# VachaLab/gorder

Hardware: AMD Instinct MI355X
Metric: trajectory frames/sec (higher is better)
Workload: dtype f32

## Files before the change

gorder_amd/csrc/gorder_hip.hip:

```cpp
#include <hip/hip_runtime.h>

#include <dlfcn.h>

#include <cmath>
#include <cstdio>
#include <cstdlib>
#include <cstring>
#include <mutex>
#include <new>
#include <string>
#include <deque>
#include <type_traits>
#include <vector>

#include "../../include/gorder_hip.h"
#include "gm_math.h"
#include "plan.h"
#include "collect_store.h"
#include "device_mem.h"
#include "replay_rows.h"
#include "leaflet_rows.h"
#include "timewise_blocks.h"
#include "ordermap_final.h"
#include "order_route.h"
// ... 135 lines not shown
    DBuf<Item> d_items_by_slot;
    DBuf<uint32_t> d_ua_item_run, d_item_run;
    DBuf<uint4> d_lgrid;
    DBuf<LocalRowPre> d_lrowpre;
    DBuf<LocalEdge> d_ledge;
    DBuf<float4> d_lfinfo;
    static constexpr uint32_t kDecidePause = 16;
    DBuf<uint32_t> d_lsummary;
    HBuf<uint32_t> h_lsummary;
    Event lsummary_written;
    bool lsummary_pending = false;
    uint32_t decide_pause = 0;
    uint64_t decide_submits = 0, decide_paused_submits = 0;
    DBuf<uint32_t> d_lneed;
    DBuf<uint2> d_ltodo;
    size_t map_lds_bytes = 0;
    bool map_staged = false;
    uint64_t map_pending = 0;
    uint32_t map_max_mol = 1;
    DBuf<u64> d_tw_sums, d_tw_cnts;
    uint64_t tw_cap = 0;
    DBuf<u64> d_twx_blocks, d_twx_rows, d_twx_totals, d_twx_edge;
    DBuf<uint32_t> d_twx_groups;
    DBuf<float> d_twx_out;
    DBuf<uint32_t> d_omx_groups;
    DBuf<float> d_omx_out;
    ExtraArgs extra{};
    DBuf<uint32_t> d_geom_group;
    DBuf<float> d_shapes;
    DBuf<float> d_inv_box;
// ... 311 lines not shown
int fold_maps(gorder_hip_handle *h) {
    if (!h->extra.maps || !h->map_pending) return GORDER_OK;
    const size_t n = (size_t)h->plan.n_acc * h->map_nx * h->map_ny;
    const uint32_t blocks = (uint32_t)std::min<size_t>((n + 255) / 256, 256 * 16);
    hipLaunchKernelGGL(k_fold_maps, dim3(blocks), dim3(256), 0, h->stream, h->d_map_packed, h->d_map_sums, h->d_map_cnts,
                       n, h->tables.leaflets.method != GORDER_LEAFLETS_NONE ? 1 : 0);
    HIP_TRY(h, hipGetLastError());
    h->map_pending = 0;
    return GORDER_OK;
}

int launch_cell_list(gorder_hip_handle *h, const LocalArgs &lo, uint32_t ns, uint32_t n_list, void *counts, size_t count_bytes) {
    const bool three = h->sw.local_three_kernels;
    TIMING_MARK(h, n_list <= kLocalBuildMax && !three ? "k_local_build" : "k_local_bin + k_local_scan + k_local_scatter");
    if (n_list <= kLocalBuildMax && !three) {
        if (n_list <= 2u * 8192u) hipLaunchKernelGGL(k_local_build<2>, dim3(ns), dim3(1024), kLocalBuildLds, h->stream, lo);
        else if (n_list <= 5u * 8192u) hipLaunchKernelGGL(k_local_build<5>, dim3(ns), dim3(1024), kLocalBuildLds, h->stream, lo);
        else hipLaunchKernelGGL(k_local_build<kLocalBuildTrips>, dim3(ns), dim3(1024), kLocalBuildLds, h->stream, lo);
        return GORDER_OK;
    }
    HIP_TRY(h, hipMemsetAsync(counts, 0, count_bytes, h->stream));
    const dim3 ga((n_list + 255) / 256, ns);
    hipLaunchKernelGGL(k_local_bin, ga, dim3(256), 0, h->stream, lo);
    hipLaunchKernelGGL(k_local_scan, dim3(ns), dim3(1024), 0, h->stream, lo);
    hipLaunchKernelGGL(k_local_scatter, ga, dim3(256), 0, h->stream, lo);
    return GORDER_OK;
}

int run_dynamic_normals(gorder_hip_handle *h, const FrameArgs &a) {
    int st;
    const uint32_t n_mol = h->plan.n_mol_total;
    if ((st = ensure(h, h->d_dyn_normals, (size_t)a.n_frames * n_mol)) != GORDER_OK) return st;
    const gorder_dynamic_normal_t &dn = h->tables.dynamic_normal;
// ... 961 lines not shown
    const size_t nm = t->leaflets.n_membrane, ncell = (size_t)kLocalMaxCells1D * kLocalMaxCells1D;
    const size_t sl = h->local_slab = local_slab_frames(nm, h->sw.local_slab);
    ST_TRY(local_build_attributes(h));
    h->local_halo = t->handle_pbc && !h->sw.local_atoms_only;
    h->local_rec_stride = (h->local_halo ? 2u : 1u) * nm;
    ST_TRY(allocate(h, h->d_lcell_of, sl * nm));
    ST_TRY(allocate(h, h->d_ltrig, sl * h->local_rec_stride * (sizeof(LocalRec) / sizeof(float))));
    ST_TRY(allocate(h, h->d_lcell_count, sl * (ncell + 1)));
    ST_TRY(allocate(h, h->d_lcell_fill, sl * ncell));
    ST_TRY(allocate(h, h->d_lgrid, sl));
    if (!h->local_halo) return GORDER_OK;
    const size_t row_cells = sl * (size_t)kLocalMaxCells1D * (kLocalMaxCells1D + 1u);
    ST_TRY(allocate(h, h->d_lrowpre, row_cells));
    ST_TRY(allocate(h, h->d_ledge, row_cells));
    ST_TRY(allocate(h, h->d_lfinfo, sl));
    ST_TRY(allocate(h, h->d_lneed, sl + 1));
    ST_TRY(allocate(h, h->d_lsummary, 2, 0));
    ST_TRY(allocate(h, h->h_lsummary, 2));
    h->h_lsummary[0] = h->h_lsummary[1] = 0u;
    HIP_TRY(h, h->lsummary_written.create());
    HIP_TRY(h, hipFuncSetAttribute(reinterpret_cast<const void *>(k_local_decide), hipFuncAttributeMaxDynamicSharedMemorySize, (int)kDecideLds));
    HIP_TRY(h, hipFuncSetAttribute(reinterpret_cast<const void *>(k_local_sums), hipFuncAttributeMaxDynamicSharedMemorySize, (int)kSumsLds));
    return allocate(h, h->d_ltodo, 1 + sl * (size_t)(p.n_mol_total ? p.n_mol_total : 1));
}

int gorder_hip_create(const gorder_tables_t *t, gorder_hip_handle **out) {
    if (!t || !out) return GORDER_ERR_INVALID_ARGUMENT;
    *out = nullptr;
    int n_dev = 0;
    if (hipGetDeviceCount(&n_dev) != hipSuccess || n_dev <= 0) return GORDER_ERR_NO_DEVICE;
    if (t->device < 0 || t->device >= n_dev) return GORDER_ERR_INVALID_ARGUMENT;
// ... 344 lines not shown
    return d;
}

static int launch_local_slabs(gorder_hip_handle *h, LocalArgs lo, uint32_t n_assign, uint32_t row0, bool report) {
    const size_t ncell = (size_t)kLocalMaxCells1D * kLocalMaxCells1D;
    for (size_t done = 0; done < n_assign; done += h->local_slab) {
        const uint32_t ns = (uint32_t)std::min<size_t>(n_assign - done, h->local_slab);
        lo.aframes = h->d_aframes + done;
        lo.n_slab = ns;
        lo.row0 = row0 + (uint32_t)done;
        lo.write_dist_frame = (done + ns == n_assign) ? (int)ns - 1 : -1;
        lo.summary_host = report && done + ns == n_assign ? h->h_lsummary : nullptr;
        if (lo.n_membrane > kLocalBuildMax || h->sw.local_three_kernels)
            HIP_TRY(h, hipMemsetAsync(h->d_lcell_fill, 0, ns * ncell * sizeof(uint32_t), h->stream));
        if (lo.sums) {
            HIP_TRY(h, hipMemsetAsync(h->d_lneed, 0, (ns + 1) * sizeof(uint32_t), h->stream));
            TIMING_MARK(h, "k_local_sums");
            hipLaunchKernelGGL(k_local_sums, dim3(ns), dim3(1024), kSumsLds, h->stream, lo);
            TIMING_MARK(h, "k_local_decide");
            hipLaunchKernelGGL(k_local_decide, dim3(ns), dim3(1024), kDecideLds, h->stream, lo);
        }
        ST_TRY(launch_cell_list(h, lo, ns, lo.n_membrane, h->d_lcell_count, ns * (ncell + 1) * sizeof(uint32_t)));
        if (lo.halo) {
            TIMING_MARK(h, "k_local_rowprefix");
            hipLaunchKernelGGL(k_local_rowprefix, dim3(kLocalMaxCells1D / 4u, ns), dim3(256), 0, h->stream, lo);
            lo.rows_groups = (lo.n_mol_total + 15u) / 16u;
            if (lo.need && !lo.sums) {
                TIMING_MARK(h, "k_local_decide");
                hipLaunchKernelGGL(k_local_decide, dim3(ns), dim3(1024), kDecideLds, h->stream, lo);
            }
            TIMING_MARK(h, "k_local_flags_rows");
            if (lo.need) hipLaunchKernelGGL(k_local_flags_rows_open, dim3(lo.rows_groups * 8u * kRowsSlots), dim3(256), 0, h->stream, lo);
            else hipLaunchKernelGGL(k_local_flags_rows, dim3(lo.rows_groups * ((ns + 7u) / 8u * 8u)), dim3(256), 0, h->stream, lo);
            TIMING_MARK(h, "k_local_flags_todo");
            hipLaunchKernelGGL(k_local_flags_todo, dim3(512), dim3(256), 0, h->stream, lo);
        } else {
            TIMING_MARK(h, "k_local_flags");
            hipLaunchKernelGGL(k_local_flags, dim3((lo.n_mol_total + 3) / 4, ns), dim3(256), 0, h->stream, lo);
        }
    }
// ... 12 lines not shown
    lo.radius_thr = local_radius_threshold(lf.radius);
    lo.cell_of = h->d_lcell_of; lo.trig = h->d_ltrig; lo.cell_count = h->d_lcell_count;
    lo.cell_fill = h->d_lcell_fill; lo.err = la.err;
    lo.grid = h->d_lgrid;
    lo.halo = h->local_halo ? 1 : 0;
    lo.prune = h->sw.local_no_prune ? 0 : (h->sw.local_decide_nothing ? 2 : 1);
    lo.rec_stride = (uint32_t)h->local_rec_stride;
    lo.rowpre = h->d_lrowpre;
    lo.edge = h->d_ledge;
    lo.finfo = h->d_lfinfo;
    lo.todo = h->d_ltodo;
    const LocalDecisions d = local_decisions(h, lo);
    lo.need = d.decide ? h->d_lneed : nullptr;
    lo.sums = d.sums ? 1 : 0;
    lo.summary = d.report ? h->d_lsummary : nullptr;
    ST_TRY(launch_local_slabs(h, lo, la.n_assign, la.row0, d.report));
    if (d.report) {
        HIP_TRY(h, hipEventRecord(h->lsummary_written, h->stream));
        h->lsummary_pending = true;
    }
    return GORDER_OK;
}

static int run_leaflets(gorder_hip_handle *h, const float *d_xyz, const float *d_box,
                        const std::vector<uint32_t> &aframes, uint32_t row0, const uint8_t *skip = nullptr) {
    if (aframes.empty()) return GORDER_OK;
    ST_TRY(upload_if_changed(h, h->d_aframes, h->up_aframes, h->up_aframes_valid, aframes));
    const gorder_leaflets_t &lf = h->tables.leaflets;
    LeafletArgs la{};
    la.xyz = d_xyz; la.box9 = d_box; la.n_atoms = h->plan.n_atoms;
// ... 1252 lines not shown
int gorder_hip_collected_normals(gorder_hip_handle *h, float *normals, uint64_t *frames, uint64_t capacity_rows, uint64_t *n_rows) {
    if (!h || !n_rows) return GORDER_ERR_INVALID_ARGUMENT;
    *n_rows = 0;
    if (!(h->collect & GORDER_COLLECT_NORMALS)) return fail(h, GORDER_ERR_INVALID_ARGUMENT, "gorder_hip_collected_normals: normals are not being collected");
    const gorder::CollectStore &store = h->collect_normals;
    *n_rows = store.n_rows();
    if ((normals || frames) && capacity_rows < store.n_rows()) return fail(h, GORDER_ERR_INVALID_ARGUMENT, "gorder_hip_collected_normals: capacity_rows is too small");
    ST_TRY(gorder_hip_synchronize(h));
    const size_t row_floats = (size_t)h->plan.n_mol_total * 3u;
    if (normals)
        store.for_each_row([&](uint64_t r, const void *row) { memcpy(normals + r * row_floats, row, row_floats * sizeof(float)); });
    if (frames && store.n_rows()) memcpy(frames, store.frames().data(), store.n_rows() * sizeof(uint64_t));
    return GORDER_OK;
}

int gorder_hip_leaflet_distances(gorder_hip_handle *h, float *dist) {
    if (!h || !dist || !h->d_adist) return GORDER_ERR_INVALID_ARGUMENT;
    ST_TRY(gorder_hip_synchronize(h));
    HIP_TRY(h, hipMemcpy(dist, h->d_adist, sizeof(float) * h->plan.n_mol_total, hipMemcpyDeviceToHost));
    return GORDER_OK;
}

int gorder_hip_spherical_stats(gorder_hip_handle *h, float out[12]) {
    if (!h || !out || h->tables.leaflets.method != GORDER_LEAFLETS_SPHERICAL || !h->d_sph_stats) return GORDER_ERR_INVALID_ARGUMENT;
    if (!h->have_assignment) return fail(h, GORDER_ERR_INVALID_ARGUMENT, "gorder_hip_spherical_stats: no assignment frame yet");
    ST_TRY(gorder_hip_synchronize(h));
    HIP_TRY(h, hipMemcpy(out, h->d_sph_stats, 12 * sizeof(float), hipMemcpyDeviceToHost));
    return GORDER_OK;
}

int gorder_hip_clustering_stats(gorder_hip_handle *h, float out[12]) {
    if (!h || !out || h->tables.leaflets.method != GORDER_LEAFLETS_CLUSTERING || !h->d_cl_stats) return GORDER_ERR_INVALID_ARGUMENT;
    if (!h->have_assignment) return fail(h, GORDER_ERR_INVALID_ARGUMENT, "gorder_hip_clustering_stats: no assignment frame yet");
// ... 74 lines not shown
    h->mol_batch_log.clear();
    h->collect_locked = false;
    h->have_assignment = false;
    h->cl_have_carry = false;
    h->replay_have_carry = false;
    h->assignment_frame = 0;
    h->manual_frames = 0;
    h->err_index = 0;
    h->err_msg.clear();
    if (h->d_own) {
        spec_poll(h, true);
        h->spec_enabled = true;
        h->spec_batches = h->spec_fixed = h->spec_exact_frames = 0;
        HIP_TRY(h, hipMemsetAsync(h->d_spec_counters, 0, 4 * sizeof(uint32_t), h->stream));
    }
    if (h->d_lsummary) {
        if (h->lsummary_pending) { (void)hipEventSynchronize(h->lsummary_written); h->lsummary_pending = false; }
        h->decide_pause = 0;
        h->decide_submits = h->decide_paused_submits = 0;
        h->h_lsummary[0] = h->h_lsummary[1] = 0u;
        HIP_TRY(h, hipMemsetAsync(h->d_lsummary, 0, 2 * sizeof(uint32_t), h->stream));
    }
    return GORDER_OK;
}

int gorder_hip_comm_unique_id(uint8_t id[128]) {
    if (!id) return GORDER_ERR_INVALID_ARGUMENT;
    RcclApi *api = rccl_api(nullptr);
    if (!api) return GORDER_ERR_DEVICE;
    UniqueId u;
// ... 152 lines not shown
```

gorder_amd/csrc/kernels_leaflets.h:

```cpp
#pragma once

namespace {

struct LeafletArgs {
    const float *xyz;
    const float *box9;
    uint32_t n_atoms;
    const uint32_t *aframes;
    uint32_t row0;
    uint8_t *aflags;
    float *adist;
    uint32_t n_mol_total;
    const uint32_t *heads;
    const uint32_t *membrane;
    uint32_t n_membrane;
    const uint32_t *methyl_begin;
    const uint32_t *methyl_atoms;
    uint32_t dim;
    int flip, pbc;
    uint32_t *err;
    const uint8_t *skip;
    uint32_t n_assign;
};

// ... 539 lines not shown
    float *trig;
    uint32_t *cell_count;
    uint32_t *cell_fill;
    int halo;
    int prune;
    uint32_t rows_groups;
    uint32_t rec_stride;
    LocalEdge *edge;
    LocalRowPre *rowpre;
    float4 *finfo;
    uint2 *todo;
    int sums;
    uint32_t *summary;
    uint32_t *summary_host;
    uint32_t *need;
    uint32_t *err;
};

constexpr uint32_t kLocalFine = 4;
constexpr uint32_t kLocalFineRows = 7;
__device__ __forceinline__ void local_axis(float L, float radius, uint32_t &nc, uint32_t &k, uint32_t k_max = kLocalFine,
                                           uint32_t nc_max = kLocalMaxCells1D) {
    nc = 1; k = 0;
    for (uint32_t kk = k_max; kk >= 1u; kk--) {
        const float fine = floorf(L / (radius / (float)kk) * 0.9999f);
        if (fine >= (float)(2u * kk + 1u) && fine <= (float)nc_max) { nc = (uint32_t)fine; k = kk; return; }
    }
}
__device__ __forceinline__ void local_grid(const LocalArgs &a, const float *box, uint32_t &nca, uint32_t &ncb,
                                           int &da, int &db, uint32_t &ka, uint32_t &kb) {
    da = (int)((a.dim + 1u) % 3u);
// ... 252 lines not shown
        if (qb == qa) break;
    }
}
__device__ __forceinline__ void local_finfo_merge(const LocalArgs &a, uint32_t s, float zlo, float zhi, uint32_t nf) {
    wave_minmax_or_bfly(zlo, zhi, nf);
    if ((threadIdx.x & 63u) == 0u) {
        uint32_t *fi = reinterpret_cast<uint32_t *>(a.finfo + s);
        if (zlo <= zhi) {
            atomicMin(fi, local_float_key(zlo));
            atomicMax(fi + 1, local_float_key(zhi));
        }
        if (nf) atomicOr(fi + 2, 1u);
    }
}
constexpr uint32_t kRowPrefixPiece = 256;
__global__ __launch_bounds__(256) void k_local_rowprefix(LocalArgs a) {
    __shared__ alignas(16) float l_c[4][kRowPrefixPiece + 4], l_s[4][kRowPrefixPiece + 4], l_q[4][kRowPrefixPiece + 4];
    __shared__ alignas(16) double l_z[4][kRowPrefixPiece + 2];
    const uint32_t s = blockIdx.y, wave = threadIdx.x >> 6, ra = blockIdx.x * 4u + wave;
    const uint4 g = a.grid[s];
    const uint32_t nca = g.x, ncs = local_row_stride(a, g.y, g.w);
    if (a.sums) {
        if (a.need[a.n_slab] == 0u || a.need[s] == 0u) return;
    } else if (blockIdx.x == 0 && s == 0 && threadIdx.x == 0) a.todo[0] = make_uint2(0u, 0u);
    if (!a.sums && blockIdx.x == 0 && threadIdx.x == 0 && a.need) {
        a.need[s] = 0u;
        if (s == 0) a.need[a.n_slab] = 0u;
    }
    if (ra >= nca) return;
    const bool merge = reinterpret_cast<const uint4 *>(a.finfo)[s].w != 2u;
    const uint32_t *cstart = a.cell_count + (size_t)s * (kLocalMaxCells1D * kLocalMaxCells1D + 1u);
    const LocalRec *rec = reinterpret_cast<const LocalRec *>(a.trig) + (size_t)s * a.rec_stride;
    float box[3];
    frame_box(a, a.aframes ? a.aframes[s] : a.frame0 + s, box);
    LocalRowPre *out = a.rowpre + (size_t)s * (kLocalMaxCells1D * (kLocalMaxCells1D + 1u)) + (size_t)ra * (ncs + 1u);
    LocalEdge *out_edge = a.edge + (size_t)s * (kLocalMaxCells1D * (kLocalMaxCells1D + 1u)) + (size_t)ra * (ncs + 1u);
    float zlo = 3.0e38f, zhi = -3.0e38f;
    uint32_t nf = 0;
    local_row_prefix<kRowPrefixPiece>(cstart, rec, out, out_edge, ra, ncs, 1.0f / box[a.dim], 0.5f * box[a.dim], l_c[wave], l_s[wave], l_z[wave],
                                      l_q[wave], zlo, zhi, nf);
    if (merge) local_finfo_merge(a, s, zlo, zhi, nf);
}

constexpr uint32_t kLocalBuildMax = 65536;
constexpr uint32_t kLocalBuildLds = 2u * kLocalMaxCells1D * kLocalMaxCells1D * (uint32_t)sizeof(uint32_t);
constexpr uint32_t kLocalBuildTrips = kLocalBuildMax / (8u * 1024u);
template <uint32_t TRIPS>
__global__ __launch_bounds__(1024) void k_local_build(LocalArgs a) {
    extern __shared__ uint32_t l_build[];
    __shared__ uint32_t l_wave[16];
    __shared__ uint32_t l_over;
    uint32_t *l_start = l_build, *l_fill = l_build + kLocalMaxCells1D * kLocalMaxCells1D;
    const uint32_t s = blockIdx.x, tid = threadIdx.x;
    if (a.sums && (a.need[a.n_slab] == 0u || a.need[s] == 0u)) return;
    const uint32_t f = a.aframes ? a.aframes[s] : a.frame0 + s;
    float box[3];
    frame_box(a, f, box);
    uint32_t nca, ncb, ka, kb;
    int da, db;
    local_grid(a, box, nca, ncb, da, db, ka, kb);
    const uint32_t ncs = local_row_stride(a, ncb, kb), ncell = nca * ncs;
    const uint32_t n_halo = a.halo ? 2u * kb : 0u;
    const int dn = (int)a.dim;
    for (uint32_t k = tid; k < ncell; k += 1024u) { l_start[k] = 0; l_fill[k] = 0; }
    if (tid == 0) l_over = 0;
    __syncthreads();
    const float *x = a.xyz + (size_t)f * a.n_atoms * 3u;
    int bad = 0;
    bool in_halo = false;
    const float inv_a = a.pbc ? (float)nca / box[da] : 0.0f, inv_b = a.pbc ? (float)ncb / box[db] : 0.0f;
    auto cell_ab = [&](float xa, float xb) -> uint32_t {
        in_halo = false;
        if (!a.pbc) return 0u;
        const float La = box[da], Lb = box[db];
        float wa = xa > La ? xa - La : xa, wb = xb > Lb ? xb - Lb : xb;
        wa = wa < 0.0f ? wa + La : wa;
        wb = wb < 0.0f ? wb + Lb : wb;
        if (__builtin_expect(!(wa >= 0.0f && wa <= La && wb >= 0.0f && wb <= Lb), 0)) {
            wa = gm_wrap(xa, La, bad);
            wb = gm_wrap(xb, Lb, bad);
        }
        const uint32_t ca = (uint32_t)fminf(fmaxf(floorf(wa * inv_a), 0.0f), (float)(nca - 1u));
        const uint32_t cb = (uint32_t)fminf(fmaxf(floorf(wb * inv_b), 0.0f), (float)(ncb - 1u));
        in_halo = cb < n_halo;
        return ca * ncs + cb;
    };
    constexpr uint32_t U = 8;
    uint32_t place[TRIPS][2], place2[TRIPS][2];
    uint32_t cells[TRIPS][4];
    bool over = false;
#pragma unroll
    for (uint32_t trip = 0; trip < TRIPS; trip++) {
        const uint32_t i0 = tid + trip * U * 1024u;
        place[trip][0] = place[trip][1] = place2[trip][0] = place2[trip][1] = 0u;
        cells[trip][0] = cells[trip][1] = cells[trip][2] = cells[trip][3] = 0u;
        if (trip * U * 1024u >= a.n_membrane) continue;
        uint32_t at[U];
        float pa[U], pb[U];
#pragma unroll
        for (uint32_t u = 0; u < U; u++) { const uint32_t i = min(i0 + u * 1024u, a.n_membrane - 1u); at[u] = a.membrane ? a.membrane[i] : i; }
#pragma unroll
        for (uint32_t u = 0; u < U; u++) { pa[u] = x[3u * (size_t)at[u] + da]; pb[u] = x[3u * (size_t)at[u] + db]; }
#pragma unroll
        for (uint32_t u = 0; u < U; u++)
            if (i0 + u * 1024u < a.n_membrane) {
                const uint32_t c = cell_ab(pa[u], pb[u]);
                cells[trip][u >> 1] |= (c | (in_halo ? 0x4000u : 0u)) << (16u * (u & 1u));
                const uint32_t r = atomicAdd(&l_start[c], 1u);
                over |= r > 255u;
                place[trip][u >> 2] |= (r & 255u) << (8u * (u & 3u));
                if (in_halo) {
                    const uint32_t r2 = atomicAdd(&l_start[c + ncb], 1u);
                    over |= r2 > 255u;
                    place2[trip][u >> 2] |= (r2 & 255u) << (8u * (u & 3u));
                }
            }
    }
    if (over) l_over = 1u;
    __syncthreads();
    const bool use_fill = l_over != 0u;
    {
        constexpr uint32_t PER = kLocalMaxCells1D * kLocalMaxCells1D / 1024u;
        const uint32_t c0 = tid * PER;
        uint32_t cnt[PER], sum = 0;
#pragma unroll
        for (uint32_t k = 0; k < PER; k++) {
            cnt[k] = c0 + k < ncell ? l_start[c0 + k] : 0u;
            sum += cnt[k];
        }
        const uint32_t incl = wave_scan_shfl(sum, tid & 63u);
        if ((tid & 63u) == 63u) l_wave[tid >> 6] = incl;
        __syncthreads();
        uint32_t run = incl - sum;
        for (uint32_t w = 0; w < (tid >> 6); w++) run += l_wave[w];
        uint32_t *cstart = a.cell_count + (size_t)s * (kLocalMaxCells1D * kLocalMaxCells1D + 1u);
#pragma unroll
        for (uint32_t k = 0; k < PER; k++) {
            if (c0 + k <= ncell) {
                cstart[c0 + k] = run;
                if (c0 + k < ncell) l_start[c0 + k] = run;
            }
            run += cnt[k];
        }
        if (tid == 1023u && c0 + PER == ncell) cstart[ncell] = run;
    }
    if (tid == 0 && a.grid) { a.grid[s] = make_uint4(nca, ncb, ka, kb); local_finfo_init(a, s); }
    __syncthreads();
    LocalRec *rec = reinterpret_cast<LocalRec *>(a.trig) + (size_t)s * a.rec_stride;
    float zlo = 3.0e38f, zhi = -3.0e38f;
    uint32_t nf = 0;
#pragma unroll
    for (uint32_t trip = 0; trip < TRIPS; trip++) {
        const uint32_t i0 = tid + trip * U * 1024u;
        if (trip * U * 1024u >= a.n_membrane) continue;
        uint32_t at[U];
        float pa[U], pb[U], pn[U];
#pragma unroll
        for (uint32_t u = 0; u < U; u++) { const uint32_t i = min(i0 + u * 1024u, a.n_membrane - 1u); at[u] = a.membrane ? a.membrane[i] : i; }
#pragma unroll
        for (uint32_t u = 0; u < U; u++) {
            pa[u] = x[3u * (size_t)at[u] + da]; pb[u] = x[3u * (size_t)at[u] + db]; pn[u] = x[3u * (size_t)at[u] + dn];
        }
#pragma unroll
        for (uint32_t u = 0; u < U; u++) {
            if (i0 + u * 1024u >= a.n_membrane) continue;
            const uint32_t cw = (cells[trip][u >> 1] >> (16u * (u & 1u))) & 0xffffu;
            const uint32_t c = cw & 0x3fffu;
            in_halo = (cw & 0x4000u) != 0u;
            const uint32_t q = l_start[c] + (use_fill ? atomicAdd(&l_fill[c], 1u) : (place[trip][u >> 2] >> (8u * (u & 3u))) & 255u);
            rec[q] = LocalRec{pa[u], pb[u], pn[u]};
            zlo = fminf(zlo, pn[u]);
            zhi = fmaxf(zhi, pn[u]);
            nf |= ((pa[u] - pa[u]) + (pb[u] - pb[u])) + (pn[u] - pn[u]) == 0.0f ? 0u : 1u;
            if (in_halo) {
                const uint32_t q2 = l_start[c + ncb] + (use_fill ? atomicAdd(&l_fill[c + ncb], 1u) : (place2[trip][u >> 2] >> (8u * (u & 3u))) & 255u);
                rec[q2] = LocalRec{pa[u], pb[u], pn[u]};
            }
        }
    }
    if (bad) raise_box_range(a.err, f);
    if (a.finfo) {
        __shared__ float l_zlo[16], l_zhi[16];
        __shared__ uint32_t l_nf[16];
        block_finfo_record(zlo, zhi, nf, ~0u, l_zlo, l_zhi, l_nf, reinterpret_cast<uint4 *>(a.finfo) + s);
    }
}

__host__ __device__ inline float local_radius_threshold(float r) {
    if (!(r > 0.0f)) return 0.0f;
    float thr = r * r;
    for (int i = 0; i < 8 && sqrtf(thr) < r; i++) thr = nextafterf(thr, INFINITY);
    for (int i = 0; i < 8; i++) {
        const float p = nextafterf(thr, 0.0f);
        if (!(p < thr) || !(sqrtf(p) >= r)) break;
        thr = p;
    }
    return thr;
}

// ... 451 lines not shown
        a.todo[1u + at] = make_uint2(s, m);
    }
}
constexpr uint32_t kRowsSlots = 1;
__global__ __launch_bounds__(256) void k_local_flags_rows(LocalArgs a) {
    __shared__ LocalRingLists l_ring[16];
    const uint32_t n_groups = a.rows_groups, linear = blockIdx.x;
    const uint32_t xcd = linear & 7u, k = linear >> 3;
    const uint32_t s = (k / n_groups) * 8u + xcd, bx = k - (k / n_groups) * n_groups;
    if (s < a.n_slab) local_rows_group(a, s, bx, l_ring);
}
__global__ __launch_bounds__(256) void k_local_flags_rows_open(LocalArgs a) {
    __shared__ LocalRingLists l_ring[16];
    const uint32_t n_groups = a.rows_groups, linear = blockIdx.x;
    const uint32_t xcd = linear & 7u, k = linear >> 3;
    if (a.need[a.n_slab] == 0u) return;
    const uint32_t slot = k / n_groups, bx = k - slot * n_groups, lane = threadIdx.x & 63u;
    uint32_t seen = 0;
    for (uint32_t base = xcd; base < a.n_slab; base += 8u * 64u) {
        const uint32_t sl = base + 8u * lane;
        uint64_t open = __ballot(sl < a.n_slab && a.need[sl] != 0u);
        while (open != 0ull) {
            const uint32_t bit = (uint32_t)__builtin_ctzll(open);
            open &= open - 1ull;
            if (seen++ % kRowsSlots == slot) local_rows_group(a, (uint32_t)__builtin_amdgcn_readfirstlane((int)(base + 8u * bit)), bx, l_ring);
        }
    }
}

constexpr uint32_t kSumsCells = 9000;
constexpr uint32_t kSumsLds = kSumsCells * 2u * (uint32_t)sizeof(unsigned long long);
struct LocalWrapped { float a, b; int bad; };
// ... 193 lines not shown
    const float mid = T - 0.5f * A, rad = 0.5005f * __builtin_amdgcn_sqrtf(fr * B);
    const float slack = 0.1f + fn * (1.05e-3f + 1e-6f * fn * Ln);
    const float r_c = __builtin_amdgcn_sqrtf(c_c * c_c + c_s * c_s);
    const float est_c = (local_atan2_fast(-c_s, -c_c) + 3.1415927f) * (Ln * 0.15915494f);
    const float shift_c = gm_min_image(hn_pos - est_c, Ln, bad);
    const float e_c = fr + 1.0f + 0.004f * fn;
    const float xr = e_c * __builtin_amdgcn_rcpf(r_c);
    const float emargin = 1e-4f * Ln + (xr + 0.5708f * xr * xr * xr) * (0.15916f * Ln);
    const bool same_image = e_c < r_c && ulo_g + shift_c > -halfn + emargin && uhi_g + shift_c < halfn - emargin;
    const bool head_near = __builtin_fabsf(mid) + rad < (halfn - 1e-3f * Ln) * fi;
    centre_above = mid > 0.0f;
    return !redo && spans_ok && c_n > r_n && same_image && head_near && a.prune != 2 &&
           __builtin_fabsf(mid) > rad + slack;
}
template <typename EdgePtr>
__device__ __forceinline__ void local_decide_frame(const LocalArgs &a, const DecideFrame &F, uint32_t s, uint32_t f, EdgePtr edge) {
    int bad = 0;
    uint32_t n_open = 0;
    for (uint32_t m0 = threadIdx.x & ~63u; m0 < a.n_mol_total; m0 += 1024u) {
        const uint32_t m_raw = m0 + (threadIdx.x & 63u);
        const bool head_ok = m_raw < a.n_mol_total;
        const uint32_t m = head_ok ? m_raw : a.n_mol_total - 1u;
        bool centre_above;
        const bool decided = local_decide_head(a, F, f, m, edge, centre_above, bad);
        if (decided && head_ok)
            a.aflags[(size_t)(a.row0 + s) * a.n_mol_total + m] = (uint8_t)((centre_above ? 1 : 0) ^ (a.flip ? 1 : 0));
        n_open += (uint32_t)__popcll(__ballot(!decided && head_ok));
    }
    if (n_open != 0u && (threadIdx.x & 63u) == 0u) { atomicAdd(&a.need[s], n_open); a.need[a.n_slab] = 1u; }
    if (bad) raise_box_range(a.err, f);
}
__global__ __launch_bounds__(1024) void k_local_decide(LocalArgs a) {
    extern __shared__ LocalEdge l_edge[];
    const uint32_t s = blockIdx.x;
    const uint32_t f = a.aframes ? a.aframes[s] : a.frame0 + s;
    float box[3];
    frame_box(a, f, box);
    const uint4 g = a.grid[s];
    const uint4 fk = reinterpret_cast<const uint4 *>(a.finfo)[s];
    DecideFrame F;
    F.nca = g.x; F.ncb = g.y; F.ka = g.z; F.kb = g.w; F.ncs = g.y + 2u * g.w; F.n_rows = 2u * g.z + 1u;
    F.da = (int)((a.dim + 1u) % 3u); F.db = (int)((a.dim + 2u) % 3u); F.dn = (int)a.dim;
    F.La = box[F.da]; F.Lb = box[F.db]; F.Ln = box[F.dn];
    F.z_min = local_key_float(fk.x); F.z_max = local_key_float(fk.y);
    const bool fail = !(F.ka >= 1u && F.kb >= 1u && F.n_rows <= 16u && fk.z == 0u && fk.x <= fk.y);
    if (a.sums && s == 0u && threadIdx.x == 0u) a.todo[0] = make_uint2(0u, 0u);
    if (fail || !(F.z_max - F.z_min < 0.75f * F.Ln) || (int)s == a.write_dist_frame || (a.sums && a.need[s] != 0u)) {
        if (threadIdx.x == 0u) { atomicAdd(&a.need[s], 1u); a.need[a.n_slab] = 1u; }
        return;
    }
    const LocalEdge *edge = a.edge + (size_t)s * (kLocalMaxCells1D * (kLocalMaxCells1D + 1u));
    const uint32_t n_entries = F.nca * (F.ncs + 1u);
    if (n_entries <= kDecideEntries) {
        const uint4 *src = reinterpret_cast<const uint4 *>(edge);
        uint4 *dst = reinterpret_cast<uint4 *>(l_edge);
        for (uint32_t i = threadIdx.x; i < n_entries; i += 1024u) dst[i] = src[i];
        __syncthreads();
        local_decide_frame<const LocalEdge *>(a, F, s, f, l_edge);
    } else {
        local_decide_frame<const LocalEdge *>(a, F, s, f, edge);
    }
}

__global__ __launch_bounds__(256) void k_local_flags_todo(LocalArgs a) {
    if (a.need && a.summary && blockIdx.x == 0u && threadIdx.x < 64u) {
        uint32_t c = 0;
        for (uint32_t s = threadIdx.x; s < a.n_slab; s += 64u) c += a.need[s] != 0u ? 1u : 0u;
        c = wave_sum_rows(c);
        if (threadIdx.x == 0u) {
            const uint32_t open = atomicAdd(&a.summary[0], c) + c, seen = atomicAdd(&a.summary[1], a.n_slab) + a.n_slab;
            if (a.summary_host) {
                a.summary_host[0] = open;
                a.summary_host[1] = seen;
                a.summary[0] = a.summary[1] = 0u;
            }
        }
    }
    const uint32_t n = a.todo[0].x;
    for (uint32_t i = blockIdx.x * 4u + (threadIdx.x >> 6); i < n; i += gridDim.x * 4u) {
        const uint2 e = a.todo[1u + i];
        local_flags_head(a, (uint32_t)__builtin_amdgcn_readfirstlane((int)e.x), (uint32_t)__builtin_amdgcn_readfirstlane((int)e.y));
    }
}

// ... 251 lines not shown
```

Before: 20.96 million.

## Compact open frames into a worklist and defer last-frame distance computation

The decide kernel now appends frames that still need work to a compact list, and the build, rowprefix and rows kernels loop over that list with a capped grid instead of launching one block per slab frame and early-exiting. The last frame of each slab is no longer forced through the full path just to produce leaflet distances. Its coordinates and box are snapshotted on device, and the distances are recomputed lazily only when the host asks for them. This cuts idle blocks and redundant full-path work per batch, at the cost of extra state, a coordinate copy per batch, and added complexity in the query path.

```diff
diff --git a/gorder_amd/csrc/gorder_hip.hip b/gorder_amd/csrc/gorder_hip.hip
--- a/gorder_amd/csrc/gorder_hip.hip
+++ b/gorder_amd/csrc/gorder_hip.hip
@@ -173,6 +173,11 @@
     uint64_t decide_submits = 0, decide_paused_submits = 0;
     DBuf<uint32_t> d_lneed;
     DBuf<uint2> d_ltodo;
+    DBuf<float> d_lkeep_xyz, d_lkeep_box;
+    DBuf<uint32_t> d_lkeep_state, d_lkeep_err;
+    DBuf<uint8_t> d_lkeep_flags;
+    LocalArgs lkeep_args{};
+    bool ldist_maybe_owed = false;
     size_t map_lds_bytes = 0;
     bool map_staged = false;
     uint64_t map_pending = 0;
@@ -514,9 +519,10 @@
     const bool three = h->sw.local_three_kernels;
     TIMING_MARK(h, n_list <= kLocalBuildMax && !three ? "k_local_build" : "k_local_bin + k_local_scan + k_local_scatter");
     if (n_list <= kLocalBuildMax && !three) {
-        if (n_list <= 2u * 8192u) hipLaunchKernelGGL(k_local_build<2>, dim3(ns), dim3(1024), kLocalBuildLds, h->stream, lo);
-        else if (n_list <= 5u * 8192u) hipLaunchKernelGGL(k_local_build<5>, dim3(ns), dim3(1024), kLocalBuildLds, h->stream, lo);
-        else hipLaunchKernelGGL(k_local_build<kLocalBuildTrips>, dim3(ns), dim3(1024), kLocalBuildLds, h->stream, lo);
+        const dim3 grid(lo.open ? std::min(ns, kOpenBuildGroups) : ns);
+        if (n_list <= 2u * 8192u) hipLaunchKernelGGL(k_local_build<2>, grid, dim3(1024), kLocalBuildLds, h->stream, lo);
+        else if (n_list <= 5u * 8192u) hipLaunchKernelGGL(k_local_build<5>, grid, dim3(1024), kLocalBuildLds, h->stream, lo);
+        else hipLaunchKernelGGL(k_local_build<kLocalBuildTrips>, grid, dim3(1024), kLocalBuildLds, h->stream, lo);
         return GORDER_OK;
     }
     HIP_TRY(h, hipMemsetAsync(counts, 0, count_bytes, h->stream));
@@ -1508,7 +1514,12 @@
     ST_TRY(allocate(h, h->d_lrowpre, row_cells));
     ST_TRY(allocate(h, h->d_ledge, row_cells));
     ST_TRY(allocate(h, h->d_lfinfo, sl));
-    ST_TRY(allocate(h, h->d_lneed, sl + 1));
+    ST_TRY(allocate(h, h->d_lneed, 2 * sl + 2));
+    ST_TRY(allocate(h, h->d_lkeep_xyz, (size_t)p.n_atoms * 3u));
+    ST_TRY(allocate(h, h->d_lkeep_box, 9, 0));
+    ST_TRY(allocate(h, h->d_lkeep_state, 1, 0));
+    ST_TRY(allocate(h, h->d_lkeep_err, kErrWords, 0xff));
+    ST_TRY(allocate(h, h->d_lkeep_flags, p.n_mol_total ? p.n_mol_total : 1));
     ST_TRY(allocate(h, h->d_lsummary, 2, 0));
     ST_TRY(allocate(h, h->h_lsummary, 2));
     h->h_lsummary[0] = h->h_lsummary[1] = 0u;
@@ -1883,7 +1894,8 @@
         if (lo.n_membrane > kLocalBuildMax || h->sw.local_three_kernels)
             HIP_TRY(h, hipMemsetAsync(h->d_lcell_fill, 0, ns * ncell * sizeof(uint32_t), h->stream));
         if (lo.sums) {
-            HIP_TRY(h, hipMemsetAsync(h->d_lneed, 0, (ns + 1) * sizeof(uint32_t), h->stream));
+            lo.open = h->d_lneed + ns + 1;
+            HIP_TRY(h, hipMemsetAsync(h->d_lneed, 0, (ns + 2) * sizeof(uint32_t), h->stream));
             TIMING_MARK(h, "k_local_sums");
             hipLaunchKernelGGL(k_local_sums, dim3(ns), dim3(1024), kSumsLds, h->stream, lo);
             TIMING_MARK(h, "k_local_decide");
@@ -1892,7 +1904,8 @@
         ST_TRY(launch_cell_list(h, lo, ns, lo.n_membrane, h->d_lcell_count, ns * (ncell + 1) * sizeof(uint32_t)));
         if (lo.halo) {
             TIMING_MARK(h, "k_local_rowprefix");
-            hipLaunchKernelGGL(k_local_rowprefix, dim3(kLocalMaxCells1D / 4u, ns), dim3(256), 0, h->stream, lo);
+            hipLaunchKernelGGL(k_local_rowprefix, dim3(kLocalMaxCells1D / 4u, lo.open ? std::min(ns, kOpenPrefixRows) : ns), dim3(256), 0,
+                               h->stream, lo);
             lo.rows_groups = (lo.n_mol_total + 15u) / 16u;
             if (lo.need && !lo.sums) {
                 TIMING_MARK(h, "k_local_decide");
@@ -1935,6 +1948,10 @@
     lo.need = d.decide ? h->d_lneed : nullptr;
     lo.sums = d.sums ? 1 : 0;
     lo.summary = d.report ? h->d_lsummary : nullptr;
+    const bool keep = d.decide && lo.adist && lo.n_membrane <= kLocalBuildMax && !h->sw.local_three_kernels;
+    if (keep) { lo.keep_xyz = h->d_lkeep_xyz; lo.keep_box = h->d_lkeep_box; lo.keep_state = h->d_lkeep_state; }
+    h->ldist_maybe_owed = keep;
+    h->lkeep_args = lo;
     ST_TRY(launch_local_slabs(h, lo, la.n_assign, la.row0, d.report));
     if (d.report) {
         HIP_TRY(h, hipEventRecord(h->lsummary_written, h->stream));
@@ -3217,9 +3234,38 @@
     return GORDER_OK;
 }
 
+static int local_owed_distances(gorder_hip_handle *h) {
+    if (!h->ldist_maybe_owed) return GORDER_OK;
+    h->ldist_maybe_owed = false;
+    uint32_t owed = 0;
+    HIP_TRY(h, hipMemcpy(&owed, h->d_lkeep_state, sizeof(owed), hipMemcpyDeviceToHost));
+    if (!owed) return GORDER_OK;
+    LocalArgs lo = h->lkeep_args;
+    lo.xyz = h->d_lkeep_xyz; lo.box9 = h->d_lkeep_box;
+    lo.aframes = nullptr; lo.frame0 = 0; lo.n_slab = 1; lo.row0 = 0;
+    lo.aflags = h->d_lkeep_flags; lo.err = h->d_lkeep_err;
+    lo.write_dist_frame = 0;
+    lo.need = nullptr; lo.open = nullptr; lo.sums = 0; lo.summary = nullptr; lo.summary_host = nullptr;
+    lo.keep_xyz = lo.keep_box = nullptr; lo.keep_state = nullptr;
+    lo.rows_groups = (lo.n_mol_total + 15u) / 16u;
+    const bool timing_on = h->timing_on;
+    h->timing_on = false;
+    const int st = launch_cell_list(h, lo, 1, lo.n_membrane, nullptr, 0);
+    h->timing_on = timing_on;
+    if (st != GORDER_OK) return st;
+    hipLaunchKernelGGL(k_local_rowprefix, dim3(kLocalMaxCells1D / 4u, 1), dim3(256), 0, h->stream, lo);
+    hipLaunchKernelGGL(k_local_flags_rows, dim3(lo.rows_groups * 8u), dim3(256), 0, h->stream, lo);
+    hipLaunchKernelGGL(k_local_flags_todo, dim3(512), dim3(256), 0, h->stream, lo);
+    HIP_TRY(h, hipGetLastError());
+    HIP_TRY(h, hipMemsetAsync(h->d_lkeep_state, 0, sizeof(uint32_t), h->stream));
+    HIP_TRY(h, hipStreamSynchronize(h->stream));
+    return GORDER_OK;
+}
+
 int gorder_hip_leaflet_distances(gorder_hip_handle *h, float *dist) {
     if (!h || !dist || !h->d_adist) return GORDER_ERR_INVALID_ARGUMENT;
     ST_TRY(gorder_hip_synchronize(h));
+    ST_TRY(local_owed_distances(h));
     HIP_TRY(h, hipMemcpy(dist, h->d_adist, sizeof(float) * h->plan.n_mol_total, hipMemcpyDeviceToHost));
     return GORDER_OK;
 }
@@ -3324,6 +3370,7 @@
         h->spec_batches = h->spec_fixed = h->spec_exact_frames = 0;
         HIP_TRY(h, hipMemsetAsync(h->d_spec_counters, 0, 4 * sizeof(uint32_t), h->stream));
     }
+    h->ldist_maybe_owed = false;
     if (h->d_lsummary) {
         if (h->lsummary_pending) { (void)hipEventSynchronize(h->lsummary_written); h->lsummary_pending = false; }
         h->decide_pause = 0;
diff --git a/gorder_amd/csrc/kernels_leaflets.h b/gorder_amd/csrc/kernels_leaflets.h
--- a/gorder_amd/csrc/kernels_leaflets.h
+++ b/gorder_amd/csrc/kernels_leaflets.h
@@ -577,7 +577,11 @@
     uint32_t *summary;
     uint32_t *summary_host;
     uint32_t *need;
+    uint32_t *open;
     uint32_t *err;
+    float *keep_xyz;
+    float *keep_box;
+    uint32_t *keep_state;
 };
 
 constexpr uint32_t kLocalFine = 4;
@@ -860,32 +864,37 @@
     }
 }
 constexpr uint32_t kRowPrefixPiece = 256;
+constexpr uint32_t kOpenBuildGroups = 256;
+constexpr uint32_t kOpenPrefixRows = 128;
 __global__ __launch_bounds__(256) void k_local_rowprefix(LocalArgs a) {
     __shared__ alignas(16) float l_c[4][kRowPrefixPiece + 4], l_s[4][kRowPrefixPiece + 4], l_q[4][kRowPrefixPiece + 4];
     __shared__ alignas(16) double l_z[4][kRowPrefixPiece + 2];
-    const uint32_t s = blockIdx.y, wave = threadIdx.x >> 6, ra = blockIdx.x * 4u + wave;
-    const uint4 g = a.grid[s];
-    const uint32_t nca = g.x, ncs = local_row_stride(a, g.y, g.w);
-    if (a.sums) {
-        if (a.need[a.n_slab] == 0u || a.need[s] == 0u) return;
-    } else if (blockIdx.x == 0 && s == 0 && threadIdx.x == 0) a.todo[0] = make_uint2(0u, 0u);
-    if (!a.sums && blockIdx.x == 0 && threadIdx.x == 0 && a.need) {
-        a.need[s] = 0u;
-        if (s == 0) a.need[a.n_slab] = 0u;
-    }
-    if (ra >= nca) return;
-    const bool merge = reinterpret_cast<const uint4 *>(a.finfo)[s].w != 2u;
-    const uint32_t *cstart = a.cell_count + (size_t)s * (kLocalMaxCells1D * kLocalMaxCells1D + 1u);
-    const LocalRec *rec = reinterpret_cast<const LocalRec *>(a.trig) + (size_t)s * a.rec_stride;
-    float box[3];
-    frame_box(a, a.aframes ? a.aframes[s] : a.frame0 + s, box);
-    LocalRowPre *out = a.rowpre + (size_t)s * (kLocalMaxCells1D * (kLocalMaxCells1D + 1u)) + (size_t)ra * (ncs + 1u);
-    LocalEdge *out_edge = a.edge + (size_t)s * (kLocalMaxCells1D * (kLocalMaxCells1D + 1u)) + (size_t)ra * (ncs + 1u);
-    float zlo = 3.0e38f, zhi = -3.0e38f;
-    uint32_t nf = 0;
-    local_row_prefix<kRowPrefixPiece>(cstart, rec, out, out_edge, ra, ncs, 1.0f / box[a.dim], 0.5f * box[a.dim], l_c[wave], l_s[wave], l_z[wave],
-                                      l_q[wave], zlo, zhi, nf);
-    if (merge) local_finfo_merge(a, s, zlo, zhi, nf);
+    const uint32_t wave = threadIdx.x >> 6, ra = blockIdx.x * 4u + wave;
+    const uint32_t n = a.open ? a.open[0] : a.n_slab;
+    for (uint32_t q = blockIdx.y; q < n; q += gridDim.y) {
+        const uint32_t s = a.open ? a.open[1u + q] : q;
+        const uint4 g = a.grid[s];
+        const uint32_t nca = g.x, ncs = local_row_stride(a, g.y, g.w);
+        if (!a.sums && blockIdx.x == 0 && s == 0 && threadIdx.x == 0) a.todo[0] = make_uint2(0u, 0u);
+        if (!a.sums && blockIdx.x == 0 && threadIdx.x == 0 && a.need) {
+            a.need[s] = 0u;
+            if (s == 0) a.need[a.n_slab] = 0u;
+        }
+        if (ra >= nca) continue;
+        const bool merge = reinterpret_cast<const uint4 *>(a.finfo)[s].w != 2u;
+        const uint32_t *cstart = a.cell_count + (size_t)s * (kLocalMaxCells1D * kLocalMaxCells1D + 1u);
+        const LocalRec *rec = reinterpret_cast<const LocalRec *>(a.trig) + (size_t)s * a.rec_stride;
+        float box[3];
+        frame_box(a, a.aframes ? a.aframes[s] : a.frame0 + s, box);
+        LocalRowPre *out = a.rowpre + (size_t)s * (kLocalMaxCells1D * (kLocalMaxCells1D + 1u)) + (size_t)ra * (ncs + 1u);
+        LocalEdge *out_edge = a.edge + (size_t)s * (kLocalMaxCells1D * (kLocalMaxCells1D + 1u)) + (size_t)ra * (ncs + 1u);
+        float zlo = 3.0e38f, zhi = -3.0e38f;
+        uint32_t nf = 0;
+        local_row_prefix<kRowPrefixPiece>(cstart, rec, out, out_edge, ra, ncs, 1.0f / box[a.dim], 0.5f * box[a.dim], l_c[wave], l_s[wave], l_z[wave],
+                                          l_q[wave], zlo, zhi, nf);
+        if (merge) local_finfo_merge(a, s, zlo, zhi, nf);
+        __builtin_amdgcn_wave_barrier();
+    }
 }
 
 constexpr uint32_t kLocalBuildMax = 65536;
@@ -897,138 +906,142 @@
     __shared__ uint32_t l_wave[16];
     __shared__ uint32_t l_over;
     uint32_t *l_start = l_build, *l_fill = l_build + kLocalMaxCells1D * kLocalMaxCells1D;
-    const uint32_t s = blockIdx.x, tid = threadIdx.x;
-    if (a.sums && (a.need[a.n_slab] == 0u || a.need[s] == 0u)) return;
-    const uint32_t f = a.aframes ? a.aframes[s] : a.frame0 + s;
-    float box[3];
-    frame_box(a, f, box);
-    uint32_t nca, ncb, ka, kb;
-    int da, db;
-    local_grid(a, box, nca, ncb, da, db, ka, kb);
-    const uint32_t ncs = local_row_stride(a, ncb, kb), ncell = nca * ncs;
-    const uint32_t n_halo = a.halo ? 2u * kb : 0u;
-    const int dn = (int)a.dim;
-    for (uint32_t k = tid; k < ncell; k += 1024u) { l_start[k] = 0; l_fill[k] = 0; }
-    if (tid == 0) l_over = 0;
-    __syncthreads();
-    const float *x = a.xyz + (size_t)f * a.n_atoms * 3u;
-    int bad = 0;
-    bool in_halo = false;
-    const float inv_a = a.pbc ? (float)nca / box[da] : 0.0f, inv_b = a.pbc ? (float)ncb / box[db] : 0.0f;
-    auto cell_ab = [&](float xa, float xb) -> uint32_t {
-        in_halo = false;
-        if (!a.pbc) return 0u;
-        const float La = box[da], Lb = box[db];
-        float wa = xa > La ? xa - La : xa, wb = xb > Lb ? xb - Lb : xb;
-        wa = wa < 0.0f ? wa + La : wa;
-        wb = wb < 0.0f ? wb + Lb : wb;
-        if (__builtin_expect(!(wa >= 0.0f && wa <= La && wb >= 0.0f && wb <= Lb), 0)) {
-            wa = gm_wrap(xa, La, bad);
-            wb = gm_wrap(xb, Lb, bad);
-        }
-        const uint32_t ca = (uint32_t)fminf(fmaxf(floorf(wa * inv_a), 0.0f), (float)(nca - 1u));
-        const uint32_t cb = (uint32_t)fminf(fmaxf(floorf(wb * inv_b), 0.0f), (float)(ncb - 1u));
-        in_halo = cb < n_halo;
-        return ca * ncs + cb;
-    };
-    constexpr uint32_t U = 8;
-    uint32_t place[TRIPS][2], place2[TRIPS][2];
-    uint32_t cells[TRIPS][4];
-    bool over = false;
-#pragma unroll
-    for (uint32_t trip = 0; trip < TRIPS; trip++) {
-        const uint32_t i0 = tid + trip * U * 1024u;
-        place[trip][0] = place[trip][1] = place2[trip][0] = place2[trip][1] = 0u;
-        cells[trip][0] = cells[trip][1] = cells[trip][2] = cells[trip][3] = 0u;
-        if (trip * U * 1024u >= a.n_membrane) continue;
-        uint32_t at[U];
-        float pa[U], pb[U];
-#pragma unroll
-        for (uint32_t u = 0; u < U; u++) { const uint32_t i = min(i0 + u * 1024u, a.n_membrane - 1u); at[u] = a.membrane ? a.membrane[i] : i; }
-#pragma unroll
-        for (uint32_t u = 0; u < U; u++) { pa[u] = x[3u * (size_t)at[u] + da]; pb[u] = x[3u * (size_t)at[u] + db]; }
-#pragma unroll
-        for (uint32_t u = 0; u < U; u++)
-            if (i0 + u * 1024u < a.n_membrane) {
-                const uint32_t c = cell_ab(pa[u], pb[u]);
-                cells[trip][u >> 1] |= (c | (in_halo ? 0x4000u : 0u)) << (16u * (u & 1u));
-                const uint32_t r = atomicAdd(&l_start[c], 1u);
-                over |= r > 255u;
-                place[trip][u >> 2] |= (r & 255u) << (8u * (u & 3u));
+    const uint32_t tid = threadIdx.x;
+    const uint32_t n_frames = a.open ? a.open[0] : a.n_slab;
+    for (uint32_t q_frame = blockIdx.x; q_frame < n_frames; q_frame += gridDim.x) {
+        const uint32_t s = a.open ? a.open[1u + q_frame] : q_frame;
+        const uint32_t f = a.aframes ? a.aframes[s] : a.frame0 + s;
+        float box[3];
+        frame_box(a, f, box);
+        uint32_t nca, ncb, ka, kb;
+        int da, db;
+        local_grid(a, box, nca, ncb, da, db, ka, kb);
+        const uint32_t ncs = local_row_stride(a, ncb, kb), ncell = nca * ncs;
+        const uint32_t n_halo = a.halo ? 2u * kb : 0u;
+        const int dn = (int)a.dim;
+        for (uint32_t k = tid; k < ncell; k += 1024u) { l_start[k] = 0; l_fill[k] = 0; }
+        if (tid == 0) l_over = 0;
+        __syncthreads();
+        const float *x = a.xyz + (size_t)f * a.n_atoms * 3u;
+        int bad = 0;
+        bool in_halo = false;
+        const float inv_a = a.pbc ? (float)nca / box[da] : 0.0f, inv_b = a.pbc ? (float)ncb / box[db] : 0.0f;
+        auto cell_ab = [&](float xa, float xb) -> uint32_t {
+            in_halo = false;
+            if (!a.pbc) return 0u;
+            const float La = box[da], Lb = box[db];
+            float wa = xa > La ? xa - La : xa, wb = xb > Lb ? xb - Lb : xb;
+            wa = wa < 0.0f ? wa + La : wa;
+            wb = wb < 0.0f ? wb + Lb : wb;
+            if (__builtin_expect(!(wa >= 0.0f && wa <= La && wb >= 0.0f && wb <= Lb), 0)) {
+                wa = gm_wrap(xa, La, bad);
+                wb = gm_wrap(xb, Lb, bad);
+            }
+            const uint32_t ca = (uint32_t)fminf(fmaxf(floorf(wa * inv_a), 0.0f), (float)(nca - 1u));
+            const uint32_t cb = (uint32_t)fminf(fmaxf(floorf(wb * inv_b), 0.0f), (float)(ncb - 1u));
+            in_halo = cb < n_halo;
+            return ca * ncs + cb;
+        };
+        constexpr uint32_t U = 8;
+        uint32_t place[TRIPS][2], place2[TRIPS][2];
+        uint32_t cells[TRIPS][4];
+        bool over = false;
+#pragma unroll
+        for (uint32_t trip = 0; trip < TRIPS; trip++) {
+            const uint32_t i0 = tid + trip * U * 1024u;
+            place[trip][0] = place[trip][1] = place2[trip][0] = place2[trip][1] = 0u;
+            cells[trip][0] = cells[trip][1] = cells[trip][2] = cells[trip][3] = 0u;
+            if (trip * U * 1024u >= a.n_membrane) continue;
+            uint32_t at[U];
+            float pa[U], pb[U];
+#pragma unroll
+            for (uint32_t u = 0; u < U; u++) { const uint32_t i = min(i0 + u * 1024u, a.n_membrane - 1u); at[u] = a.membrane ? a.membrane[i] : i; }
+#pragma unroll
+            for (uint32_t u = 0; u < U; u++) { pa[u] = x[3u * (size_t)at[u] + da]; pb[u] = x[3u * (size_t)at[u] + db]; }
+#pragma unroll
+            for (uint32_t u = 0; u < U; u++)
+                if (i0 + u * 1024u < a.n_membrane) {
+                    const uint32_t c = cell_ab(pa[u], pb[u]);
+                    cells[trip][u >> 1] |= (c | (in_halo ? 0x4000u : 0u)) << (16u * (u & 1u));
+                    const uint32_t r = atomicAdd(&l_start[c], 1u);
+                    over |= r > 255u;
+                    place[trip][u >> 2] |= (r & 255u) << (8u * (u & 3u));
+                    if (in_halo) {
+                        const uint32_t r2 = atomicAdd(&l_start[c + ncb], 1u);
+                        over |= r2 > 255u;
+                        place2[trip][u >> 2] |= (r2 & 255u) << (8u * (u & 3u));
+                    }
+                }
+        }
+        if (over) l_over = 1u;
+        __syncthreads();
+        const bool use_fill = l_over != 0u;
+        {
+            constexpr uint32_t PER = kLocalMaxCells1D * kLocalMaxCells1D / 1024u;
+            const uint32_t c0 = tid * PER;
+            uint32_t cnt[PER], sum = 0;
+#pragma unroll
+            for (uint32_t k = 0; k < PER; k++) {
+                cnt[k] = c0 + k < ncell ? l_start[c0 + k] : 0u;
+                sum += cnt[k];
+            }
+            const uint32_t incl = wave_scan_shfl(sum, tid & 63u);
+            if ((tid & 63u) == 63u) l_wave[tid >> 6] = incl;
+            __syncthreads();
+            uint32_t run = incl - sum;
+            for (uint32_t w = 0; w < (tid >> 6); w++) run += l_wave[w];
+            uint32_t *cstart = a.cell_count + (size_t)s * (kLocalMaxCells1D * kLocalMaxCells1D + 1u);
+#pragma unroll
+            for (uint32_t k = 0; k < PER; k++) {
+                if (c0 + k <= ncell) {
+                    cstart[c0 + k] = run;
+                    if (c0 + k < ncell) l_start[c0 + k] = run;
+                }
+                run += cnt[k];
+            }
+            if (tid == 1023u && c0 + PER == ncell) cstart[ncell] = run;
+        }
+        if (tid == 0 && a.grid) { a.grid[s] = make_uint4(nca, ncb, ka, kb); local_finfo_init(a, s); }
+        __syncthreads();
+        LocalRec *rec = reinterpret_cast<LocalRec *>(a.trig) + (size_t)s * a.rec_stride;
+        float zlo = 3.0e38f, zhi = -3.0e38f;
+        uint32_t nf = 0;
+#pragma unroll
+        for (uint32_t trip = 0; trip < TRIPS; trip++) {
+            const uint32_t i0 = tid + trip * U * 1024u;
+            if (trip * U * 1024u >= a.n_membrane) continue;
+            uint32_t at[U];
+            float pa[U], pb[U], pn[U];
+#pragma unroll
+            for (uint32_t u = 0; u < U; u++) { const uint32_t i = min(i0 + u * 1024u, a.n_membrane - 1u); at[u] = a.membrane ? a.membrane[i] : i; }
+#pragma unroll
+            for (uint32_t u = 0; u < U; u++) {
+                pa[u] = x[3u * (size_t)at[u] + da]; pb[u] = x[3u * (size_t)at[u] + db]; pn[u] = x[3u * (size_t)at[u] + dn];
+            }
+#pragma unroll
+            for (uint32_t u = 0; u < U; u++) {
+                if (i0 + u * 1024u >= a.n_membrane) continue;
+                const uint32_t cw = (cells[trip][u >> 1] >> (16u * (u & 1u))) & 0xffffu;
+                const uint32_t c = cw & 0x3fffu;
+                in_halo = (cw & 0x4000u) != 0u;
+                const uint32_t q = l_start[c] + (use_fill ? atomicAdd(&l_fill[c], 1u) : (place[trip][u >> 2] >> (8u * (u & 3u))) & 255u);
+                rec[q] = LocalRec{pa[u], pb[u], pn[u]};
+                zlo = fminf(zlo, pn[u]);
+                zhi = fmaxf(zhi, pn[u]);
+                nf |= ((pa[u] - pa[u]) + (pb[u] - pb[u])) + (pn[u] - pn[u]) == 0.0f ? 0u : 1u;
                 if (in_halo) {
-                    const uint32_t r2 = atomicAdd(&l_start[c + ncb], 1u);
-                    over |= r2 > 255u;
-                    place2[trip][u >> 2] |= (r2 & 255u) << (8u * (u & 3u));
+                    const uint32_t q2 = l_start[c + ncb] + (use_fill ? atomicAdd(&l_fill[c + ncb], 1u) : (place2[trip][u >> 2] >> (8u * (u & 3u))) & 255u);
+                    rec[q2] = LocalRec{pa[u], pb[u], pn[u]};
                 }
             }
-    }
-    if (over) l_over = 1u;
-    __syncthreads();
-    const bool use_fill = l_over != 0u;
-    {
-        constexpr uint32_t PER = kLocalMaxCells1D * kLocalMaxCells1D / 1024u;
-        const uint32_t c0 = tid * PER;
-        uint32_t cnt[PER], sum = 0;
-#pragma unroll
-        for (uint32_t k = 0; k < PER; k++) {
-            cnt[k] = c0 + k < ncell ? l_start[c0 + k] : 0u;
-            sum += cnt[k];
-        }
-        const uint32_t incl = wave_scan_shfl(sum, tid & 63u);
-        if ((tid & 63u) == 63u) l_wave[tid >> 6] = incl;
+        }
+        if (bad) raise_box_range(a.err, f);
+        if (a.finfo) {
+            __shared__ float l_zlo[16], l_zhi[16];
+            __shared__ uint32_t l_nf[16];
+            block_finfo_record(zlo, zhi, nf, ~0u, l_zlo, l_zhi, l_nf, reinterpret_cast<uint4 *>(a.finfo) + s);
+        }
         __syncthreads();
-        uint32_t run = incl - sum;
-        for (uint32_t w = 0; w < (tid >> 6); w++) run += l_wave[w];
-        uint32_t *cstart = a.cell_count + (size_t)s * (kLocalMaxCells1D * kLocalMaxCells1D + 1u);
-#pragma unroll
-        for (uint32_t k = 0; k < PER; k++) {
-            if (c0 + k <= ncell) {
-                cstart[c0 + k] = run;
-                if (c0 + k < ncell) l_start[c0 + k] = run;
-            }
-            run += cnt[k];
-        }
-        if (tid == 1023u && c0 + PER == ncell) cstart[ncell] = run;
-    }
-    if (tid == 0 && a.grid) { a.grid[s] = make_uint4(nca, ncb, ka, kb); local_finfo_init(a, s); }
-    __syncthreads();
-    LocalRec *rec = reinterpret_cast<LocalRec *>(a.trig) + (size_t)s * a.rec_stride;
-    float zlo = 3.0e38f, zhi = -3.0e38f;
-    uint32_t nf = 0;
-#pragma unroll
-    for (uint32_t trip = 0; trip < TRIPS; trip++) {
-        const uint32_t i0 = tid + trip * U * 1024u;
-        if (trip * U * 1024u >= a.n_membrane) continue;
-        uint32_t at[U];
-        float pa[U], pb[U], pn[U];
-#pragma unroll
-        for (uint32_t u = 0; u < U; u++) { const uint32_t i = min(i0 + u * 1024u, a.n_membrane - 1u); at[u] = a.membrane ? a.membrane[i] : i; }
-#pragma unroll
-        for (uint32_t u = 0; u < U; u++) {
-            pa[u] = x[3u * (size_t)at[u] + da]; pb[u] = x[3u * (size_t)at[u] + db]; pn[u] = x[3u * (size_t)at[u] + dn];
-        }
-#pragma unroll
-        for (uint32_t u = 0; u < U; u++) {
-            if (i0 + u * 1024u >= a.n_membrane) continue;
-            const uint32_t cw = (cells[trip][u >> 1] >> (16u * (u & 1u))) & 0xffffu;
-            const uint32_t c = cw & 0x3fffu;
-            in_halo = (cw & 0x4000u) != 0u;
-            const uint32_t q = l_start[c] + (use_fill ? atomicAdd(&l_fill[c], 1u) : (place[trip][u >> 2] >> (8u * (u & 3u))) & 255u);
-            rec[q] = LocalRec{pa[u], pb[u], pn[u]};
-            zlo = fminf(zlo, pn[u]);
-            zhi = fmaxf(zhi, pn[u]);
-            nf |= ((pa[u] - pa[u]) + (pb[u] - pb[u])) + (pn[u] - pn[u]) == 0.0f ? 0u : 1u;
-            if (in_halo) {
-                const uint32_t q2 = l_start[c + ncb] + (use_fill ? atomicAdd(&l_fill[c + ncb], 1u) : (place2[trip][u >> 2] >> (8u * (u & 3u))) & 255u);
-                rec[q2] = LocalRec{pa[u], pb[u], pn[u]};
-            }
-        }
-    }
-    if (bad) raise_box_range(a.err, f);
-    if (a.finfo) {
-        __shared__ float l_zlo[16], l_zhi[16];
-        __shared__ uint32_t l_nf[16];
-        block_finfo_record(zlo, zhi, nf, ~0u, l_zlo, l_zhi, l_nf, reinterpret_cast<uint4 *>(a.finfo) + s);
     }
 }
 
@@ -1510,8 +1523,14 @@
     __shared__ LocalRingLists l_ring[16];
     const uint32_t n_groups = a.rows_groups, linear = blockIdx.x;
     const uint32_t xcd = linear & 7u, k = linear >> 3;
+    const uint32_t slot = k / n_groups, bx = k - slot * n_groups;
+    if (a.open) {
+        const uint32_t n = a.open[0];
+        for (uint32_t q = xcd + 8u * slot; q < n; q += 8u * kRowsSlots) local_rows_group(a, a.open[1u + q], bx, l_ring);
+        return;
+    }
     if (a.need[a.n_slab] == 0u) return;
-    const uint32_t slot = k / n_groups, bx = k - slot * n_groups, lane = threadIdx.x & 63u;
+    const uint32_t lane = threadIdx.x & 63u;
     uint32_t seen = 0;
     for (uint32_t base = xcd; base < a.n_slab; base += 8u * 64u) {
         const uint32_t sl = base + 8u * lane;
@@ -1735,7 +1754,7 @@
            __builtin_fabsf(mid) > rad + slack;
 }
 template <typename EdgePtr>
-__device__ __forceinline__ void local_decide_frame(const LocalArgs &a, const DecideFrame &F, uint32_t s, uint32_t f, EdgePtr edge) {
+__device__ __forceinline__ uint32_t local_decide_frame(const LocalArgs &a, const DecideFrame &F, uint32_t s, uint32_t f, EdgePtr edge) {
     int bad = 0;
     uint32_t n_open = 0;
     for (uint32_t m0 = threadIdx.x & ~63u; m0 < a.n_mol_total; m0 += 1024u) {
@@ -1748,13 +1767,27 @@
             a.aflags[(size_t)(a.row0 + s) * a.n_mol_total + m] = (uint8_t)((centre_above ? 1 : 0) ^ (a.flip ? 1 : 0));
         n_open += (uint32_t)__popcll(__ballot(!decided && head_ok));
     }
-    if (n_open != 0u && (threadIdx.x & 63u) == 0u) { atomicAdd(&a.need[s], n_open); a.need[a.n_slab] = 1u; }
+    if (n_open != 0u && (threadIdx.x & 63u) == 0u) {
+        const uint32_t before = atomicAdd(&a.need[s], n_open);
+        a.need[a.n_slab] = 1u;
+        if (a.open && before == 0u) a.open[1u + atomicAdd(&a.open[0], 1u)] = s;
+    }
     if (bad) raise_box_range(a.err, f);
+    return n_open;
 }
 __global__ __launch_bounds__(1024) void k_local_decide(LocalArgs a) {
     extern __shared__ LocalEdge l_edge[];
     const uint32_t s = blockIdx.x;
     const uint32_t f = a.aframes ? a.aframes[s] : a.frame0 + s;
+    const bool keeps = a.keep_xyz && a.write_dist_frame >= 0;
+    const bool kept = keeps && (int)s == a.write_dist_frame;
+    if (keeps) {
+        const uint32_t fk = a.aframes ? a.aframes[a.write_dist_frame] : a.frame0 + (uint32_t)a.write_dist_frame;
+        const float *src = a.xyz + (size_t)fk * a.n_atoms * 3u;
+        const uint32_t n_words = a.n_atoms * 3u;
+        for (uint32_t i = blockIdx.x * 1024u + threadIdx.x; i < n_words; i += gridDim.x * 1024u) a.keep_xyz[i] = src[i];
+        if (kept && a.pbc && threadIdx.x < 9u) a.keep_box[threadIdx.x] = a.box9[9u * (size_t)fk + threadIdx.x];
+    }
     float box[3];
     frame_box(a, f, box);
     const uint4 g = a.grid[s];
@@ -1766,20 +1799,30 @@
     F.z_min = local_key_float(fk.x); F.z_max = local_key_float(fk.y);
     const bool fail = !(F.ka >= 1u && F.kb >= 1u && F.n_rows <= 16u && fk.z == 0u && fk.x <= fk.y);
     if (a.sums && s == 0u && threadIdx.x == 0u) a.todo[0] = make_uint2(0u, 0u);
-    if (fail || !(F.z_max - F.z_min < 0.75f * F.Ln) || (int)s == a.write_dist_frame || (a.sums && a.need[s] != 0u)) {
-        if (threadIdx.x == 0u) { atomicAdd(&a.need[s], 1u); a.need[a.n_slab] = 1u; }
+    if (fail || !(F.z_max - F.z_min < 0.75f * F.Ln) || ((int)s == a.write_dist_frame && !keeps) || (a.sums && a.need[s] != 0u)) {
+        if (threadIdx.x == 0u) {
+            atomicAdd(&a.need[s], 1u);
+            a.need[a.n_slab] = 1u;
+            if (a.open) a.open[1u + atomicAdd(&a.open[0], 1u)] = s;
+            if (kept) a.keep_state[0] = 0u;
+        }
         return;
     }
     const LocalEdge *edge = a.edge + (size_t)s * (kLocalMaxCells1D * (kLocalMaxCells1D + 1u));
     const uint32_t n_entries = F.nca * (F.ncs + 1u);
+    uint32_t n_open;
     if (n_entries <= kDecideEntries) {
         const uint4 *src = reinterpret_cast<const uint4 *>(edge);
         uint4 *dst = reinterpret_cast<uint4 *>(l_edge);
         for (uint32_t i = threadIdx.x; i < n_entries; i += 1024u) dst[i] = src[i];
         __syncthreads();
-        local_decide_frame<const LocalEdge *>(a, F, s, f, l_edge);
+        n_open = local_decide_frame<const LocalEdge *>(a, F, s, f, l_edge);
     } else {
-        local_decide_frame<const LocalEdge *>(a, F, s, f, edge);
+        n_open = local_decide_frame<const LocalEdge *>(a, F, s, f, edge);
+    }
+    if (kept) {
+        const int any_open = __syncthreads_or(n_open != 0u);
+        if (threadIdx.x == 0u) a.keep_state[0] = any_open ? 0u : 1u;
     }
 }
 
@@ -1789,6 +1832,7 @@
         for (uint32_t s = threadIdx.x; s < a.n_slab; s += 64u) c += a.need[s] != 0u ? 1u : 0u;
         c = wave_sum_rows(c);
         if (threadIdx.x == 0u) {
+            if (a.keep_state && a.write_dist_frame >= 0 && a.keep_state[0] != 0u) c += 1u;
             const uint32_t open = atomicAdd(&a.summary[0], c) + c, seen = atomicAdd(&a.summary[1], a.n_slab) + a.n_slab;
             if (a.summary_host) {
                 a.summary_host[0] = open;
```

Result: slower. 20.23 million (-3.4%).
